# automl/CARL

Measured on AMD Instinct MI355X. Metric: env-steps/sec (whole node) at 65k parallel contexts, 1/2/4/8 MI355X, higher is better.
Workload: dtype f32

## Files before the change

carl_amd/csrc/carl_policy.hip:

```cpp
#include <hip/hip_runtime.h>

#include <cstdint>

#include "../../include/carl_amd.h"
#include "classic_control.hip.h"
#include "host_common.hpp"
#include "policy_host.hpp"
#include "policy_kernels.hip.h"
#include "policy_launch.hpp"

namespace carl_host {

int policy_set_floats(const carl_policy_t* p) {
  if (p->n_in < 1 || p->n_in > CARL_POLICY_MAX_IN || p->n_out < 1 || p->n_out > 4 || p->n_hidden < 0 ||
      p->n_hidden > CARL_POLICY_MAX_HIDDEN)
    return -1;
  for (int l = 0; l < p->n_hidden; ++l)
    if (p->width[l] < 1 || p->width[l] > CARL_POLICY_MAX_WIDTH) return -1;
  const int64_t total = (int64_t)policy_transform_offset(p) + 2 * (int64_t)p->n_in + 1;
  return (int)((total + 3) / 4 * 4);
}

int policy_transform_offset(const carl_policy_t* p) {
  int total = 0, prev = p->n_in;
// ... 72 lines not shown
    return fail(CARL_ERR_INVALID_ARGUMENT, "%s: io.row_pitch %d < n_lanes %d", who, io->row_pitch, b->n_lanes);
  if (!carl_host::staged_rows(b, io, 15))
    return fail(CARL_ERR_UNSUPPORTED, "%s: rows of %d lanes for %d lanes: the closed-loop rollout writes the staged layout "
                "only (pitch %% 16 == 0 and n_lanes %% 16 == 0 or pitch == carl_rollout_pitch(n_lanes), arrays on 16-byte "
                "boundaries)", who, io->row_pitch > 0 ? io->row_pitch : b->n_lanes, b->n_lanes);
  return 0;
}

int check_batch_and_policy(const char* who, const carl_batch_t* batch, const carl_policy_t* policy_host,
                           carl_family_info_t* fi) {
  if (batch == nullptr || policy_host == nullptr) return fail(CARL_ERR_INVALID_ARGUMENT, "%s: batch / policy is NULL", who);
  if (batch->family >= CARL_N_FAMILIES)
    return fail(CARL_ERR_INVALID_ARGUMENT, "%s: family %d is a Brax family -- the closed-loop rollout covers the "
                "classic-control families only", who, batch->family);
  if (int e = validate_batch(batch, who)) return e;
  if (int e = carl_family_info(batch->family, fi)) return e;
  return validate_policy(batch, policy_host, *fi, who);
}

}

int check_rollout_policy(const char* who, const carl_batch_t* batch, const carl_policy_t* policy_host,
                         const carl_step_io_t* io, int32_t n_steps, const carl_policy_summary_t* summary_out,
                         carl_family_info_t* fi) {
  if (int e = check_batch_and_policy(who, batch, policy_host, fi)) return e;
  if (n_steps < 0) return fail(CARL_ERR_INVALID_ARGUMENT, "%s: n_steps %d < 0", who, n_steps);
  if (io == nullptr) {
    if (summary_out == nullptr || !summary_out->episodes || !summary_out->return_sum || !summary_out->length_sum)
      return fail(CARL_ERR_INVALID_ARGUMENT, "%s: summary mode (io NULL) needs all three summary arrays", who);
  } else {
    if (int e = validate_io(batch, io, *fi, who)) return e;
    if (summary_out != nullptr && (!summary_out->episodes || !summary_out->return_sum || !summary_out->length_sum))
      return fail(CARL_ERR_INVALID_ARGUMENT, "%s: a summary needs all three arrays", who);
  }
  if (summary_out != nullptr && !(batch->flags & CARL_FLAG_AUTORESET))
    return fail(CARL_ERR_UNSUPPORTED, "%s: a summary needs CARL_FLAG_AUTORESET (without auto-reset a finished lane "
                "reports done on every later step, and its episode would be counted on each of them)", who);
  return 0;
}

int policy_rollout_without_steps(const char* who, const carl_batch_t* batch, const carl_policy_summary_t* summary_out,
                                 void* stream) {
  if (summary_out == nullptr || batch->n_lanes == 0) return 0;
  hipStream_t s = (hipStream_t)stream;
  const size_t bytes = (size_t)batch->n_lanes * 4;
  for (void* p : {(void*)summary_out->episodes, (void*)summary_out->return_sum, (void*)summary_out->length_sum})
    if (const hipError_t e = hipMemsetAsync(p, 0, bytes, s); e != hipSuccess)
      return fail((int)e, "%s: hipMemsetAsync: %s", who, hipGetErrorString(e));
  return 0;
}

int check_evaluate_policy(const char* who, const carl_batch_t* batch, const carl_policy_t* policy_host,
                          int32_t n_episodes, int32_t max_steps, const carl_policy_episodes_t* out,
                          carl_family_info_t* fi) {
  if (int e = check_batch_and_policy(who, batch, policy_host, fi)) return e;
  if (out == nullptr || !out->episodes || !out->steps || !out->ret || !out->length || !out->context_id ||
      !out->terminated)
    return fail(CARL_ERR_INVALID_ARGUMENT, "%s: out and all six of its arrays are required", who);
  if (n_episodes < 1) return fail(CARL_ERR_INVALID_ARGUMENT, "%s: n_episodes %d < 1", who, n_episodes);
  if (max_steps < 0) return fail(CARL_ERR_INVALID_ARGUMENT, "%s: max_steps %d < 0", who, max_steps);
  if ((int64_t)n_episodes * batch->n_lanes >= ((int64_t)1 << 31))
    return fail(CARL_ERR_INVALID_ARGUMENT, "%s: n_episodes %d x %d lanes records do not fit 2^31 - 1", who, n_episodes,
                batch->n_lanes);
  if (!(batch->flags & CARL_FLAG_AUTORESET))
    return fail(CARL_ERR_UNSUPPORTED, "%s: needs CARL_FLAG_AUTORESET (without auto-reset a finished lane reports done on "
                "every later step, and its episode would be counted on each of them)", who);
  return 0;
}

}

namespace {

using carl_host::launch_policy_kernel;
using carl_host::PolicyKernel;
using carl_host::with_padded_hidden;

template <class Fam>
int launch_policy(const carl_batch_t* b, const carl_policy_t* p, const carl_step_io_t* io, int n_steps,
                  const carl_policy_summary_t* sum, hipStream_t s) {
  const bool summary = io == nullptr;
  static_assert(carl::policy_lds_bytes<Fam, 64, false>() + carl::static_lds_bytes<Fam>() <= carl::kCuLdsBytes,
                "the closed-loop rollout's LDS does not fit a compute unit");
  const auto k = with_padded_hidden(carl_host::policy_padded_hidden(p), [&](auto h) {
    constexpr int H = decltype(h)::value;
    if (summary) return PolicyKernel{carl::policy_rollout_kernel<Fam, H, true>, carl::policy_lds_bytes<Fam, H, true>()};
    return PolicyKernel{carl::policy_rollout_kernel<Fam, H, false>, carl::policy_lds_bytes<Fam, H, false>()};
  });
  const int threads = summary ? carl::kPolicyThreadsSummary : carl::kPolicyThreadsTransitions;
  return launch_policy_kernel("carl_rollout_policy", k, b->n_lanes, threads, s, *b, carl_host::launch_io(b, io), *p,
                              carl_host::policy_set_floats(p), carl_host::launch_summary(sum), n_steps);
}

template <class Fam>
int launch_episodes(const carl_batch_t* b, const carl_policy_t* p, int n_episodes, int max_steps,
                    const carl_policy_episodes_t* out, hipStream_t s) {
  const auto k = with_padded_hidden(carl_host::policy_padded_hidden(p), [](auto h) {
    constexpr int H = decltype(h)::value;
    return PolicyKernel{carl::policy_episodes_kernel<Fam, H>, carl::policy_lds_bytes<Fam, H, true>()};
  });
  return launch_policy_kernel("carl_evaluate_policy", k, b->n_lanes, carl::kPolicyThreadsSummary, s, *b, *p,
                              carl_host::policy_set_floats(p), *out, n_episodes, max_steps);
}

}

extern "C" {

int32_t carl_policy_lane_quantum(void) { return carl::kPolicyLanes; }

int32_t carl_policy_set_floats(const carl_policy_t* policy_host) {
  if (policy_host == nullptr) return -1;
  return carl_host::policy_set_floats(policy_host);
}

int carl_rollout_policy(const carl_batch_t* batch, const carl_policy_t* policy_host, const carl_step_io_t* io,
                        int32_t n_steps, const carl_policy_summary_t* summary_out, void* stream) {
  const char* who = "carl_rollout_policy";
  carl_family_info_t fi;
  if (int e = carl_host::check_rollout_policy(who, batch, policy_host, io, n_steps, summary_out, &fi)) return e;
  if (batch->n_lanes == 0 || n_steps == 0) return carl_host::policy_rollout_without_steps(who, batch, summary_out, stream);
  return carl_host::with_classic_family(batch, [&](auto fam) {
    return launch_policy<decltype(fam)>(batch, policy_host, io, n_steps, summary_out, (hipStream_t)stream);
  });
}

int carl_evaluate_policy(const carl_batch_t* batch, const carl_policy_t* policy_host, int32_t n_episodes,
                         int32_t max_steps, const carl_policy_episodes_t* out, void* stream) {
  carl_family_info_t fi;
  if (int e = carl_host::check_evaluate_policy("carl_evaluate_policy", batch, policy_host, n_episodes, max_steps, out, &fi))
    return e;
  if (batch->n_lanes == 0) return 0;
  return carl_host::with_classic_family(batch, [&](auto fam) {
    return launch_episodes<decltype(fam)>(batch, policy_host, n_episodes, max_steps, out, (hipStream_t)stream);
  });
}

}
```

carl_amd/csrc/carl_policy_sample.hip:

```cpp
#include <hip/hip_runtime.h>

#include <cstdint>

#include "../../include/carl_amd.h"
#include "classic_control.hip.h"
#include "host_common.hpp"
#include "policy_host.hpp"
#include "policy_kernels.hip.h"
#include "policy_launch.hpp"

namespace carl_host {

int check_sampling(const char* who, const carl_policy_sampling_t* smp, const carl_family_info_t& fi, LogProb log_prob) {
  if (smp == nullptr) return fail(CARL_ERR_INVALID_ARGUMENT, "%s: sampling is NULL", who);
  if (!fi.action_is_discrete && smp->log_std == nullptr)
    return fail(CARL_ERR_INVALID_ARGUMENT, "%s: a Box family needs sampling->log_std ([n_sets] on the device)", who);
  if (log_prob == LogProb::kRefused && smp->log_prob != nullptr)
    return fail(CARL_ERR_INVALID_ARGUMENT, "%s: sampling->log_prob is a transitions-mode output (io != NULL); this mode "
                "stores nothing per step", who);
  if (log_prob == LogProb::kRequired && smp->log_prob == nullptr)
    return fail(CARL_ERR_INVALID_ARGUMENT, "%s: a sampled launch with a critic stores the log-probabilities: "
                "sampling->log_prob is NULL", who);
  if ((reinterpret_cast<uintptr_t>(smp->log_prob) & 15) != 0)
    return fail(CARL_ERR_UNSUPPORTED, "%s: sampling->log_prob is not on a 16-byte boundary", who);
  return 0;
}

}

namespace {

using carl_host::check_sampling;
using carl_host::launch_policy_kernel;
using carl_host::LogProb;
using carl_host::PolicyKernel;
using carl_host::with_padded_hidden;

template <class Fam>
int launch_sampled(const carl_batch_t* b, const carl_policy_t* p, const carl_policy_sampling_t* smp,
                   const carl_step_io_t* io, int n_steps, const carl_policy_summary_t* sum, hipStream_t s) {
  const bool summary = io == nullptr, logp = smp->log_prob != nullptr;
  static_assert(carl::policy_lds_bytes<Fam, 64, false, true>() + carl::static_lds_bytes<Fam>() <= carl::kCuLdsBytes,
                "the sampled rollout's LDS (the log_prob column included) does not fit a compute unit");
  const auto k = with_padded_hidden(carl_host::policy_padded_hidden(p), [&](auto h) {
    constexpr int H = decltype(h)::value;
    using carl::policy_lds_bytes;
    if (summary) return PolicyKernel{carl::policy_rollout_sampled_kernel<Fam, H, true, false>, policy_lds_bytes<Fam, H, true>()};
    if (logp)
      return PolicyKernel{carl::policy_rollout_sampled_kernel<Fam, H, false, true>, policy_lds_bytes<Fam, H, false, true>()};
    return PolicyKernel{carl::policy_rollout_sampled_kernel<Fam, H, false, false>, policy_lds_bytes<Fam, H, false>()};
  });
  const int threads = summary ? carl::kPolicyThreadsSummary : carl::kPolicyThreadsTransitions;
  return launch_policy_kernel("carl_rollout_policy_sampled", k, b->n_lanes, threads, s, *b, carl_host::launch_io(b, io), *p,
                              carl_host::policy_set_floats(p), carl_host::launch_summary(sum), n_steps, *smp);
}

template <class Fam>
int launch_sampled_episodes(const carl_batch_t* b, const carl_policy_t* p, const carl_policy_sampling_t* smp,
                            int n_episodes, int max_steps, const carl_policy_episodes_t* out, hipStream_t s) {
  const auto k = with_padded_hidden(carl_host::policy_padded_hidden(p), [](auto h) {
    constexpr int H = decltype(h)::value;
    return PolicyKernel{carl::policy_episodes_sampled_kernel<Fam, H>, carl::policy_lds_bytes<Fam, H, true>()};
  });
  return launch_policy_kernel("carl_evaluate_policy_sampled", k, b->n_lanes, carl::kPolicyThreadsSummary, s, *b, *p,
                              carl_host::policy_set_floats(p), *out, n_episodes, max_steps, *smp);
}

}

extern "C" {

int carl_rollout_policy_sampled(const carl_batch_t* batch, const carl_policy_t* policy_host,
                                const carl_policy_sampling_t* sampling, const carl_step_io_t* io, int32_t n_steps,
                                const carl_policy_summary_t* summary_out, void* stream) {
  const char* who = "carl_rollout_policy_sampled";
  carl_family_info_t fi;
  if (int e = carl_host::check_rollout_policy(who, batch, policy_host, io, n_steps, summary_out, &fi)) return e;
  if (int e = check_sampling(who, sampling, fi, io != nullptr ? LogProb::kOptional : LogProb::kRefused)) return e;
  if (batch->n_lanes == 0 || n_steps == 0) return carl_host::policy_rollout_without_steps(who, batch, summary_out, stream);
  return carl_host::with_classic_family(batch, [&](auto fam) {
    return launch_sampled<decltype(fam)>(batch, policy_host, sampling, io, n_steps, summary_out, (hipStream_t)stream);
  });
}

int carl_evaluate_policy_sampled(const carl_batch_t* batch, const carl_policy_t* policy_host,
                                 const carl_policy_sampling_t* sampling, int32_t n_episodes, int32_t max_steps,
                                 const carl_policy_episodes_t* out, void* stream) {
  const char* who = "carl_evaluate_policy_sampled";
  carl_family_info_t fi;
  if (int e = carl_host::check_evaluate_policy(who, batch, policy_host, n_episodes, max_steps, out, &fi)) return e;
  if (int e = check_sampling(who, sampling, fi, LogProb::kRefused)) return e;
  if (batch->n_lanes == 0) return 0;
  return carl_host::with_classic_family(batch, [&](auto fam) {
    return launch_sampled_episodes<decltype(fam)>(batch, policy_host, sampling, n_episodes, max_steps, out,
                                                  (hipStream_t)stream);
  });
}

}
```

carl_amd/csrc/engine_kernels.hip.h:

```cpp
#pragma once

#include <type_traits>

#include "carl_device.hip.h"


namespace carl {

template <bool LDS>
using ctx_t = std::conditional_t<LDS, LdsCtx, GlobalCtx>;

template <class Fam, class = void>
struct has_tables : std::false_type {};
template <class Fam>
struct has_tables<Fam, std::void_t<decltype(Fam::kUsesSinCosTab)>> : std::bool_constant<Fam::kUsesSinCosTab> {};

template <class Fam>
__device__ __forceinline__ void stage_family_tables() {
  if constexpr (has_tables<Fam>::value) {
    Fam::stage_tables();
    __syncthreads();
  }
}

// ... 613 lines not shown
    } else if constexpr (kU8) {
      return CARL_LD(reinterpret_cast<const unsigned int*>(p));
    } else if constexpr (kF16 || kBF16) {
      return CARL_LD(reinterpret_cast<const vu2*>(p));
    } else {
      const vi4* q = reinterpret_cast<const vi4*>(p);
      return Wide{CARL_LD(q), CARL_LD(q + 1)};
    }
#undef CARL_LD
  }
  __device__ static __forceinline__ LdsRow narrow(const R& r) {
    if constexpr (kSame || kNarrow) {
      return r;
    } else {
      return V{r.lo.x, r.lo.z, r.hi.x, r.hi.z};
    }
  }

  bool fast;

  __device__ __forceinline__ void issue(const AStore* __restrict__ act, size_t n, int cols, int lane_base, int l, int t0_,
                                        int n_steps) {
    t0 = t0_;
    fast = t0 + CHUNK <= n_steps;
    if constexpr (DEEP) {
      const int lane4 = min(lane_base + 4 * l, cols - 4);
      const int last = n_steps - 1;
      a0 = load_row(act + (size_t)min(t0, last) * n + lane4);
      a1 = load_row(act + (size_t)min(t0 + 1, last) * n + lane4);
      a2 = load_row(act + (size_t)min(t0 + 2, last) * n + lane4);
      a3 = load_row(act + (size_t)min(t0 + 3, last) * n + lane4);
      if constexpr (CHUNK == 8) {
        a4 = load_row(act + (size_t)min(t0 + 4, last) * n + lane4);
        a5 = load_row(act + (size_t)min(t0 + 5, last) * n + lane4);
        a6 = load_row(act + (size_t)min(t0 + 6, last) * n + lane4);
        a7 = load_row(act + (size_t)min(t0 + 7, last) * n + lane4);
      }
      return;
    }
    if (!fast) return;
    const int lane4 = min(lane_base + 4 * l, cols - 4);
    const AStore* row = act + (size_t)t0 * n;
    a0 = load_row(row + lane4);
    row += n;
    a1 = load_row(row + lane4);
    row += n;
    a2 = load_row(row + lane4);
    row += n;
    a3 = load_row(row + lane4);
    if constexpr (CHUNK == 8) {
      row += n;
      a4 = load_row(row + lane4);
      row += n;
      a5 = load_row(row + lane4);
      row += n;
      a6 = load_row(row + lane4);
      row += n;
      a7 = load_row(row + lane4);
    }
  }
  __device__ __forceinline__ void commit(LdsElem* buf, const AStore* __restrict__ act, size_t n, int cols, int lane_base, int l,
                                         int n_steps) const {
    LdsRow* dst = reinterpret_cast<LdsRow*>(buf + 4 * l);
    constexpr int row = kRolloutLanes / 4;
    if (fast || DEEP) {
      dst[0] = narrow(a0);
      dst[row] = narrow(a1);
      dst[2 * row] = narrow(a2);
      dst[3 * row] = narrow(a3);
      if constexpr (CHUNK == 8) {
        dst[4 * row] = narrow(a4);
        dst[5 * row] = narrow(a5);
        dst[6 * row] = narrow(a6);
        dst[7 * row] = narrow(a7);
      }
      return;
    }
    const AStore* src = act + (size_t)t0 * n + min(lane_base + 4 * l, cols - 4);
#pragma unroll 1
    for (int u = 0; u < CHUNK && t0 + u < n_steps; ++u) dst[u * row] = narrow(load_row(src + (size_t)u * n));
  }
};

template <class Fam>
__device__ __forceinline__ void drain_records(char* buf, const carl_step_io_t& io, size_t n, int cols, int lane_base, int l,
                                              int which, int t0, int steps) {
  using SK = LdsSink<Fam>;
  const int valid = min(kRolloutLanes, cols - lane_base);
  typedef float vf4 __attribute__((ext_vector_type(4)));
  auto put = [](char* dst, const char* src) {
    const vf4 v = *reinterpret_cast<const vf4*>(src);
    __builtin_nontemporal_store(v, reinterpret_cast<vf4*>(dst));
  };
  for (int u = which; u < steps; u += kStorers) {
    char* rec = buf + (size_t)u * SK::kStepBytes;
    const size_t row = (size_t)(t0 + u) * n + lane_base;
    char* g_obs = reinterpret_cast<char*>(io.obs + row * Fam::D);
    char* fl = rec + SK::kFlagOff + 16 * l;
    const int fl_lane = 16 * (l & 15);
    uint8_t* fl_dst = (l < 16) ? io.terminated + row + fl_lane : io.truncated + row + fl_lane;
    if (valid == kRolloutLanes) {
#pragma unroll
      for (int off = 0; off < SK::kObsBytes; off += 1024) put(g_obs + off + 16 * l, rec + off + 16 * l);
      put(reinterpret_cast<char*>(io.reward + row) + 16 * l, rec + SK::kObsBytes + 16 * l);
      if (l < 32) put(reinterpret_cast<char*>(fl_dst), fl);
    } else {
#pragma unroll
      for (int off = 0; off < SK::kObsBytes; off += 1024)
        if (off + 16 * l < valid * Fam::D * 4) put(g_obs + off + 16 * l, rec + off + 16 * l);
      if (16 * l < valid * 4) put(reinterpret_cast<char*>(io.reward + row) + 16 * l, rec + SK::kObsBytes + 16 * l);
      if (l < 32 && fl_lane < valid) put(reinterpret_cast<char*>(fl_dst), fl);
    }
    if (l < 32) *reinterpret_cast<vf4*>(fl) = vf4{0.0f, 0.0f, 0.0f, 0.0f};
  }
}

template <class Fam, int CHUNK>
__device__ __forceinline__ void zero_flag_rows(char* out_buf, int l, int which) {
  using SK = LdsSink<Fam>;
  typedef float vf4 __attribute__((ext_vector_type(4)));
  if (l < 32)
    for (int u = which; u < 2 * CHUNK; u += kStorers)
      *reinterpret_cast<vf4*>(out_buf + (size_t)u * SK::kStepBytes + SK::kFlagOff + 16 * l) = vf4{0.0f, 0.0f, 0.0f, 0.0f};
}

template <class Fam, class Ctx>
__device__ __forceinline__ void load_staged_lane(const carl_batch_t& b, const Ctx& ctx, int lane, bool active,
                                                 LaneRegs<Fam>& r) {
  const int src = min(lane, b.n_lanes - 1);
  load_lane<Fam>(b, ctx, src, r);
  if (!r.episode_valid) {
    r.episode = b.episode[src];
    r.episode_valid = true;
    settle(r.episode);
  }
  r.valid = active;
}

template <class Fam, int A64, bool PLAIN, bool LDSCTX, bool MOVES, bool FINAL, bool AR, int CHUNK, bool DEEPALL = false>
__device__ __forceinline__ void rollout_staged_body(const carl_batch_t& b, const carl_step_io_t& io, const int n_steps,
                                                    const int wg, float* lds_dyn) {
  constexpr int kStageChunk = CHUNK;
  stage_family_tables<Fam>();
  using AStore = action_store_t<Fam, A64>;
  using Action = typename Fam::Action;
  using SK = LdsSink<Fam>;
  constexpr bool kDeep = !std::is_same_v<AStore, long long> &&
                         (DEEPALL || (deep_action_prefetch_of<Fam>::value && !std::is_same_v<AStore, Action>));
  using Pipe = ActionPipe<AStore, Action, kStageChunk, kDeep>;
  using LdsAct = typename Pipe::LdsElem;
  LdsAct* act_buf = reinterpret_cast<LdsAct*>(lds_dyn);
  char* out_buf = reinterpret_cast<char*>(lds_dyn) + (size_t)2 * kStageChunk * kRolloutLanes * sizeof(float);
  float* ctx_lds = reinterpret_cast<float*>(out_buf + (size_t)2 * kStageChunk * SK::kStepBytes);
  const ctx_t<LDSCTX> ctx = make_ctx<LDSCTX, Fam::F>(b, ctx_lds);
  const int wave = __builtin_amdgcn_readfirstlane((int)(threadIdx.x / kWave));
  const int storer = wave - (kRolloutLanes / kWave + 1);
  const bool compute = wave < kRolloutLanes / kWave;
  const bool loader = wave == kRolloutLanes / kWave;
  const int hl = threadIdx.x % kWave;
  const int lane_base = wg * kRolloutLanes;
  const int lane = lane_base + (compute ? (int)threadIdx.x : 0);
  const bool active = compute && lane < b.n_lanes;
  const uint64_t glane = (uint64_t)(b.lane_offset + lane);
  const size_t n = (size_t)io.row_pitch;
  const int n_cols = (b.n_lanes + 15) & ~15;
  const int max_steps = b.max_episode_steps;
  const AStore* act = static_cast<const AStore*>(io.action);
  constexpr int kBufActs = kStageChunk * kRolloutLanes;
  LaneRegs<Fam> r{};
  Pipe pipe;
  [[maybe_unused]] Pipe pipe_b;
  float* const final_base = (io.final_obs != nullptr && active) ? io.final_obs + (size_t)lane * Fam::D : nullptr;
  if (!compute && !loader) zero_flag_rows<Fam, CHUNK>(out_buf, hl, storer);
  if (loader) {
    pipe.issue(act, n, n_cols, lane_base, hl, 0, n_steps);
    pipe.commit(act_buf, act, n, n_cols, lane_base, hl, n_steps);
    pipe.issue(act, n, n_cols, lane_base, hl, kStageChunk, n_steps);
    if constexpr (kDeep) pipe_b.issue(act, n, n_cols, lane_base, hl, 2 * kStageChunk, n_steps);
  } else if (compute) {
    load_staged_lane<Fam>(b, ctx, lane, active, r);
  }
  __syncthreads();
  auto run_role = [&](auto role_tag) -> int {
  constexpr int ROLE = decltype(role_tag)::value;
  if constexpr (ROLE == 1 && kDeep) {
    int lbuf = 0;
    for (int t0 = 0;;) {
      pipe.commit(act_buf + (lbuf ^ 1) * kBufActs, act, n, n_cols, lane_base, hl, n_steps);
      pipe.issue(act, n, n_cols, lane_base, hl, t0 + 3 * kStageChunk, n_steps);
      __syncthreads();
      lbuf ^= 1;
      if (t0 + kStageChunk >= n_steps) break;
      pipe_b.commit(act_buf + (lbuf ^ 1) * kBufActs, act, n, n_cols, lane_base, hl, n_steps);
      pipe_b.issue(act, n, n_cols, lane_base, hl, t0 + 4 * kStageChunk, n_steps);
      __syncthreads();
      lbuf ^= 1;
      t0 += 2 * kStageChunk;
      if (t0 >= n_steps) break;
    }
    return lbuf;
  }
  int buf = 0;
  [[maybe_unused]] DenseNext<Fam> nx{};
  [[maybe_unused]] const bool autoreset = (b.flags & CARL_FLAG_AUTORESET) != 0;
  [[maybe_unused]] const int max_steps_eff = max_steps > 0 ? max_steps : 0x7fffffff;
// ... 115 lines not shown
```

carl_amd/csrc/policy_kernels.hip.h:

```cpp
#pragma once

#include "engine_kernels.hip.h"

namespace carl {

constexpr int kPolicyLanes = kRolloutLanes;
constexpr int kPolicyThreadsSummary = kPolicyLanes;
constexpr int kPolicyThreadsTransitions = kPolicyLanes + kStorers * kWave;

template <class Fam>
struct policy_outputs : std::integral_constant<int, std::is_same_v<typename Fam::Action, float> ? 1
                                                    : (std::is_same_v<Fam, CartPole> ? 2 : 3)> {};

template <class Fam, int H>
struct PolicyLayout {
  static constexpr int K = (Fam::F + Fam::D + 3) / 4 * 4;
  static constexpr int HI = H == 0 ? K : H;
  static constexpr int kW1 = 0, kB1 = kW1 + H * K, kW2 = kB1 + H, kB2 = kW2 + H * H, kWh = kB2 + H, kBh = kWh + HI * 4;
  static constexpr int kShift = kBh + 4, kScale = kShift + K, kClip = kScale + K;
  static constexpr int kFloats = kClip + 4;
  static constexpr size_t kBytes = (size_t)kFloats * sizeof(float);
};

template <bool LOGP>
__host__ __device__ constexpr size_t policy_logp_lds_bytes(int chunk) {
  return LOGP ? (size_t)2 * chunk * kPolicyLanes * 4 : 0;
}
template <class Fam, bool LOGP = false>
__host__ __device__ constexpr int policy_chunk() {
  return rollout_staged_lds_bytes<Fam, 8>() + policy_logp_lds_bytes<LOGP>(8) + PolicyLayout<Fam, 64>::kBytes +
                     static_lds_bytes<Fam>() <= kCuLdsBytes ? 8 : 4;
}
template <class Fam, int H, bool SUMMARY, bool LOGP = false>
__host__ __device__ constexpr size_t policy_lds_bytes() {
  constexpr int CHUNK = policy_chunk<Fam, LOGP>();
  return PolicyLayout<Fam, H>::kBytes +
         (SUMMARY ? 0 : rollout_staged_lds_bytes<Fam, CHUNK>() + policy_logp_lds_bytes<LOGP>(CHUNK));
}

template <class Fam, int H>
__device__ __forceinline__ void stage_policy(float* w, const carl_policy_t& pol, int set_floats, int set) {
  using L = PolicyLayout<Fam, H>;
  const float* src = pol.params + (size_t)set * set_floats;
  const int n_in = pol.n_in, n_ctx = pol.n_ctx, n_out = pol.n_out;
  const int nh = pol.n_hidden;
  const int w0 = nh > 0 ? pol.width[0] : 0, w1 = nh > 1 ? pol.width[1] : 0;
  const int dims[CARL_POLICY_MAX_HIDDEN + 2] = {n_in, nh > 0 ? w0 : n_out, nh > 1 ? w1 : n_out, n_out};
  int p_w[CARL_POLICY_MAX_HIDDEN + 1] = {0, 0, 0}, p_b[CARL_POLICY_MAX_HIDDEN + 1] = {0, 0, 0};
  int off = 0;
#pragma unroll
  for (int l = 0; l <= CARL_POLICY_MAX_HIDDEN; ++l) {
    if (l <= nh) {
      p_w[l] = off;
      off += dims[l + 1] * dims[l];
      p_b[l] = off;
      off += dims[l + 1];
    }
  }
  const int p_w0 = p_w[0], p_b0 = p_b[0], p_w1 = p_w[1], p_b1 = p_b[1];
  const int p_shift = off, p_scale = p_shift + n_in, p_clip = p_scale + n_in;
  auto in_of = [&](int s) -> int {
    if (s < n_ctx) return s;
    if (s >= Fam::F && s < Fam::F + Fam::D) return n_ctx + (s - Fam::F);
    return -1;
  };
  const int hw = p_w[nh], hb = p_b[nh], hin = dims[nh];
  for (int e = threadIdx.x; e < L::kFloats; e += blockDim.x) {
    float v = 0.0f;
    if (e < L::kB1) {
      const int j = e / L::K, s = e % L::K, i = in_of(s);
      if (j < w0 && i >= 0) v = src[p_w0 + j * n_in + i];
    } else if (e < L::kW2) {
      const int j = e - L::kB1;
      if (j < w0) v = src[p_b0 + j];
    } else if (e < L::kB2) {
      const int j = (e - L::kW2) / (H > 0 ? H : 1), i = (e - L::kW2) % (H > 0 ? H : 1);
      if (j < w1 && i < w0) v = src[p_w1 + j * w0 + i];
    } else if (e < L::kWh) {
      const int j = e - L::kB2;
      if (j < w1) v = src[p_b1 + j];
    } else if (e < L::kBh) {
      const int j = (e - L::kWh) / 4, k = (e - L::kWh) % 4;
      const int i = H == 0 ? in_of(j) : (j < hin ? j : -1);
      if (k < n_out && i >= 0) v = src[hw + k * hin + i];
    } else if (e < L::kShift) {
      const int k = e - L::kBh;
      if (k < n_out) v = src[hb + k];
    } else if (e < L::kScale) {
      const int i = in_of(e - L::kShift);
      if (i >= 0) v = src[p_shift + i];
    } else if (e < L::kClip) {
      const int i = in_of(e - L::kScale);
      if (i >= 0) v = src[p_scale + i];
    } else {
      v = src[p_clip];
    }
    w[e] = v;
  }
}

typedef float pvf4 __attribute__((ext_vector_type(4)));

__device__ __forceinline__ pvf4 bcast4(const float* p) { return *reinterpret_cast<const pvf4*>(p); }

__device__ __forceinline__ float tanh_fast(float v) {
#pragma clang fp contract(off)
  const float e = __expf(2.0f * v);
  return 1.0f - __fdividef(2.0f, e + 1.0f);
}

template <int N>
__device__ __forceinline__ void activate(float (&h)[N], int act, int width) {
  if (act == CARL_POLICY_TANH) {
#pragma unroll
    for (int j = 0; j < N; ++j) h[j] = tanh_fast(h[j]);
  } else if (act == CARL_POLICY_RELU) {
#pragma unroll
    for (int j = 0; j < N; ++j) h[j] = fmaxf(h[j], 0.0f);
  }
  if (width < N) {
// ... 89 lines not shown
    return y[0];
  } else {
    int best = 0;
    float top = y[0];
#pragma unroll
    for (int k = 1; k < policy_outputs<Fam>::value; ++k) {
      const bool gt = y[k] > top;
      best = gt ? k : best;
      top = gt ? y[k] : top;
    }
    return best;
  }
}

template <class Fam>
struct ModePick {
  static constexpr bool kSampled = false, kLogProb = false;
};

template <class Fam, bool LOGP>
struct SampledPick {
  static constexpr bool kSampled = true, kLogProb = LOGP;
  uint64_t seed;
  float sigma;
  float lp0;

  static __device__ __forceinline__ SampledPick of(const carl_policy_sampling_t& smp, const carl_policy_t& pol) {
    SampledPick p{smp.seed, 1.0f, 0.0f};
    if constexpr (std::is_same_v<typename Fam::Action, float>) {
      const float ls = smp.log_std[(int)blockIdx.x * kPolicyLanes / pol.lanes_per_set];
      p.sigma = expf(ls);
      p.lp0 = -ls - 0.918938533204672742f;
    }
    return p;
  }

  template <int H>
  __device__ __forceinline__ typename Fam::Action choose(const float* w, const float (&x)[PolicyLayout<Fam, H>::K],
                                                         int n_hidden, int act, int w0, int w1, uint64_t glane,
                                                         const LaneRegs<Fam>& r, float& lp) const {
#pragma clang fp contract(off)
    const u32x4 wd = lane_words(seed, glane, r.episode - 1u, kSubSample | (uint32_t)r.elapsed);
    float y[4];
    if constexpr (std::is_same_v<typename Fam::Action, float>) {
      const float z = normal_from_words(wd.x, wd.y);
      policy_head<Fam, H>(w, x, n_hidden, act, w0, w1, y);
      if constexpr (LOGP) lp = __fmaf_rn(-0.5f * z, z, lp0);
      return __fmaf_rn(sigma, z, y[0]);
    } else {
      constexpr int NA = policy_outputs<Fam>::value;
      const float u = u01(wd.x);
      policy_head<Fam, H>(w, x, n_hidden, act, w0, w1, y);
      float m = y[0];
#pragma unroll
      for (int k = 1; k < NA; ++k) m = fmaxf(m, y[k]);
      float c[NA];
      float s = 0.0f;
#pragma unroll
      for (int k = 0; k < NA; ++k) c[k] = s = s + expf(y[k] - m);
      const float t = u * s;
      int a = NA - 1;
      float ya = y[NA - 1];
#pragma unroll
      for (int k = NA - 2; k >= 0; --k) {
        const bool in = t < c[k];
        a = in ? k : a;
        ya = in ? y[k] : ya;
      }
      if constexpr (LOGP) lp = (ya - m) - logf(s);
      return a;
    }
  }
};

template <class Fam>
struct NullSink {
  static constexpr bool kLazyFlags = true;
  __device__ __forceinline__ void put_reward(float) const {}
  __device__ __forceinline__ void put_flags(bool, bool) const {}
  __device__ __forceinline__ void put_obs(const float (&)[Fam::D]) const {}
  __device__ __forceinline__ float* final_obs_ptr() const { return nullptr; }
};

__device__ __forceinline__ void drain_actions(const char* buf, void* action, size_t n, int cols, int lane_base, int l,
                                              int which, int t0, int steps) {
  const int valid = min(kPolicyLanes, cols - lane_base);
  for (int u = which; u < steps; u += kStorers) {
    const char* src = buf + (size_t)u * kPolicyLanes * 4 + 16 * l;
    char* dst = reinterpret_cast<char*>(action) + ((size_t)(t0 + u) * n + lane_base) * 4 + 16 * l;
    if (4 * l < valid) __builtin_nontemporal_store(*reinterpret_cast<const pvf4*>(src), reinterpret_cast<pvf4*>(dst));
  }
}

template <class Fam, int H, bool SUMMARY>
__global__ void __launch_bounds__(SUMMARY ? kPolicyThreadsSummary : kPolicyThreadsTransitions)
    policy_rollout_kernel(const carl_batch_t b, const carl_step_io_t io, const carl_policy_t pol, const int set_floats,
                          const carl_policy_summary_t sum, const int n_steps) {
  using Pick = ModePick<Fam>;
  const Pick pick{};
  float* const log_prob = nullptr;
#include "policy_rollout_body.inc"
}

template <class Fam, int H, bool SUMMARY, bool LOGP>
__global__ void __launch_bounds__(SUMMARY ? kPolicyThreadsSummary : kPolicyThreadsTransitions)
    policy_rollout_sampled_kernel(const carl_batch_t b, const carl_step_io_t io, const carl_policy_t pol,
                                  const int set_floats, const carl_policy_summary_t sum, const int n_steps,
                                  const carl_policy_sampling_t smp) {
  static_assert(!(SUMMARY && LOGP), "a summary stores no per-step column");
  using Pick = SampledPick<Fam, LOGP>;
  const Pick pick = Pick::of(smp, pol);
  float* const log_prob = smp.log_prob;
#include "policy_rollout_body.inc"
}

template <class Fam>
struct TermSink {
  static constexpr bool kLazyFlags = true;
  bool* te;
  __device__ __forceinline__ void put_reward(float) const {}
  __device__ __forceinline__ void put_flags(bool t, bool) const { *te = t; }
  __device__ __forceinline__ void put_obs(const float (&)[Fam::D]) const {}
  __device__ __forceinline__ float* final_obs_ptr() const { return nullptr; }
};

template <class Fam, int H>
struct NoInputStats {
  static constexpr bool kOn = false;
};

template <class Fam, int H>
__global__ void __launch_bounds__(kPolicyThreadsSummary)
    policy_episodes_kernel(const carl_batch_t b, const carl_policy_t pol, const int set_floats,
                           const carl_policy_episodes_t ep, const int n_episodes, const int max_steps) {
  using Pick = ModePick<Fam>;
  const Pick pick{};
  using Stats = NoInputStats<Fam, H>;
  [[maybe_unused]] Stats istats;
#include "policy_episodes_body.inc"
}

template <class Fam, int H>
__global__ void __launch_bounds__(kPolicyThreadsSummary)
    policy_episodes_sampled_kernel(const carl_batch_t b, const carl_policy_t pol, const int set_floats,
                                   const carl_policy_episodes_t ep, const int n_episodes, const int max_steps,
                                   const carl_policy_sampling_t smp) {
  using Pick = SampledPick<Fam, false>;
  const Pick pick = Pick::of(smp, pol);
  using Stats = NoInputStats<Fam, H>;
  [[maybe_unused]] Stats istats;
#include "policy_episodes_body.inc"
}

}
```

carl_amd/csrc/policy_launch.hpp:

```cpp
#pragma once

#include <hip/hip_runtime.h>

#include <cstddef>
#include <type_traits>

#include "../../include/carl_amd.h"
#include "host_common.hpp"
#include "policy_kernels.hip.h"

namespace carl_host {

template <class Fn>
auto with_padded_hidden(int H, Fn&& fn) {
  return H == 0    ? fn(std::integral_constant<int, 0>{})
         : H == 32 ? fn(std::integral_constant<int, 32>{})
                   : fn(std::integral_constant<int, 64>{});
}

template <class... P>
struct PolicyKernel {
  void (*fn)(P...);
  size_t lds;
};
template <class... P>
PolicyKernel(void (*)(P...), size_t) -> PolicyKernel<P...>;

inline int policy_workgroups(int32_t n_lanes) {
  return n_lanes <= 0 ? 0 : (n_lanes + carl::kPolicyLanes - 1) / carl::kPolicyLanes;
}

template <class... P>
int launch_policy_kernel(const char* who, PolicyKernel<P...> k, int32_t n_lanes, int threads, hipStream_t s,
                         const P&... args) {
  if (int e = ensure_dynamic_lds(reinterpret_cast<const void*>(k.fn), k.lds, who)) return e;
  hipLaunchKernelGGL(k.fn, dim3(policy_workgroups(n_lanes)), dim3(threads), k.lds, s, args...);
  return check_launch(who);
}

inline carl_step_io_t launch_io(const carl_batch_t* b, const carl_step_io_t* io) {
  carl_step_io_t r{};
  if (io != nullptr) {
    r = *io;
    r.row_pitch = io->row_pitch > 0 ? io->row_pitch : b->n_lanes;
  }
  return r;
}

inline carl_policy_summary_t launch_summary(const carl_policy_summary_t* sum) {
  return sum != nullptr ? *sum : carl_policy_summary_t{nullptr, nullptr, nullptr};
}

inline carl_policy_sampling_t launch_sampling(const carl_policy_sampling_t* smp) {
  return smp != nullptr ? *smp : carl_policy_sampling_t{0, nullptr, nullptr};
}

}
```

carl_amd/csrc/policy_rollout_body.inc:

```
  using L = PolicyLayout<Fam, H>;
  using SK = LdsSink<Fam>;
  using Action = typename Fam::Action;
  constexpr int CHUNK = policy_chunk<Fam, Pick::kLogProb>();
  extern __shared__ float lds_dyn[];
  stage_family_tables<Fam>();
  float* const wts = lds_dyn;
  char* const out_buf = reinterpret_cast<char*>(lds_dyn) + L::kBytes;
  char* const act_buf = out_buf + (size_t)2 * CHUNK * SK::kStepBytes;
  char* const lp_buf = act_buf + (size_t)2 * CHUNK * kPolicyLanes * 4;
  const int lane_base = (int)blockIdx.x * kPolicyLanes;
  stage_policy<Fam, H>(wts, pol, set_floats, lane_base / pol.lanes_per_set);
  const GlobalCtx ctx{b.ctx_table, b.ctx_stride};
  const int wave = __builtin_amdgcn_readfirstlane((int)(threadIdx.x / kWave));
  const bool compute = wave < kPolicyLanes / kWave;
  const int hl = threadIdx.x % kWave;
  const int storer = wave - kPolicyLanes / kWave;
  const int lane = lane_base + (compute ? (int)threadIdx.x : 0);
  const bool active = compute && lane < b.n_lanes;
  const uint64_t glane = (uint64_t)(b.lane_offset + lane);
  const size_t n = (size_t)io.row_pitch;
  const int n_cols = (b.n_lanes + 15) & ~15;
  if (!SUMMARY && !compute) zero_flag_rows<Fam, CHUNK>(out_buf, hl, storer);
  __syncthreads();

  if (compute) {
    LaneRegs<Fam> r{};
    load_staged_lane<Fam>(b, ctx, lane, active, r);
    float* const final_base = (!SUMMARY && io.final_obs != nullptr && active) ? io.final_obs + (size_t)lane * Fam::D : nullptr;
    const int n_ctx = pol.n_ctx, n_hidden = pol.n_hidden, act = pol.activation;
    const int w0 = pol.width[0], w1 = pol.width[1];
    const float clip = wts[L::kClip];
    float x[L::K];
#pragma unroll
    for (int s = 0; s < L::K; ++s) x[s] = 0.0f;
    int x_cidx = -1;
    int ep_count = 0, len_sum = 0;
    float ret_sum = 0.0f;
    int buf = 0;
    for (int t0 = 0; t0 < n_steps; t0 += CHUNK, buf ^= 1) {
      const int steps = min(CHUNK, n_steps - t0);
      if constexpr (predraw_of<Fam>::value) predraw<Fam>(b, glane, r);
      char* const rec = out_buf + (size_t)buf * CHUNK * SK::kStepBytes;
      Action* const my_act = reinterpret_cast<Action*>(act_buf + (size_t)buf * CHUNK * kPolicyLanes * 4) + threadIdx.x;
#pragma unroll 1
      for (int u = 0; u < steps; ++u) {
        if (ballot(r.cidx != x_cidx) != 0ull) {
#pragma unroll
          for (int k = 0; k < Fam::F; ++k)
            if (k < n_ctx) x[k] = normalize_input(ctx.get(pol.ctx_rows[k], r.cidx), wts[L::kShift + k], wts[L::kScale + k], clip);
          x_cidx = r.cidx;
        }
        float o[Fam::D];
        Fam::observe(r.s, r.aux, o);
#pragma unroll
        for (int d = 0; d < Fam::D; ++d)
          x[Fam::F + d] = normalize_input(o[d], wts[L::kShift + Fam::F + d], wts[L::kScale + Fam::F + d], clip);
        [[maybe_unused]] float lp;
        Action a;
        if constexpr (Pick::kSampled)
          a = pick.template choose<H>(wts, x, n_hidden, act, w0, w1, glane, r, lp);
        else
          a = policy_action<Fam, H>(wts, x, n_hidden, act, w0, w1);
        const int before = r.n_new_episodes;
        if constexpr (SUMMARY) {
          step_lane<Fam, GlobalCtx, true, NullSink<Fam>>(b, ctx, NullSink<Fam>{}, b.max_episode_steps, true, lane, glane,
                                                          a, r);
        } else {
          my_act[u * kPolicyLanes] = a;
          if constexpr (Pick::kLogProb)
            reinterpret_cast<float*>(lp_buf + (size_t)buf * CHUNK * kPolicyLanes * 4)[u * kPolicyLanes + threadIdx.x] = lp;
          const SK sink{rec + (size_t)u * SK::kStepBytes, final_base, n * Fam::D, t0 + u, (int)threadIdx.x};
          step_lane<Fam, GlobalCtx, true, SK>(b, ctx, sink, b.max_episode_steps, true, lane, glane, a, r);
        }
        const bool fin = r.n_new_episodes != before;
        ep_count += fin ? 1 : 0;
        len_sum += fin ? r.fin_length : 0;
        ret_sum = fin ? ret_sum + r.fin_return : ret_sum;
      }
      if constexpr (!SUMMARY) __syncthreads();
    }
    if (active) {
      store_lane<Fam>(b, ctx, lane, r);
      if (sum.episodes != nullptr) {
        sum.episodes[lane] = ep_count;
        sum.return_sum[lane] = ret_sum;
        sum.length_sum[lane] = len_sum;
      }
    }
  } else if constexpr (!SUMMARY) {
    int buf = 0;
    for (int t0 = 0; t0 < n_steps; t0 += CHUNK, buf ^= 1) {
      if (t0 > 0) {
        drain_records<Fam>(out_buf + (size_t)(buf ^ 1) * CHUNK * SK::kStepBytes, io, n, n_cols, lane_base, hl, storer,
                           t0 - CHUNK, CHUNK);
        drain_actions(act_buf + (size_t)(buf ^ 1) * CHUNK * kPolicyLanes * 4, const_cast<void*>(io.action), n, n_cols,
                      lane_base, hl, storer, t0 - CHUNK, CHUNK);
        if constexpr (Pick::kLogProb)
          drain_actions(lp_buf + (size_t)(buf ^ 1) * CHUNK * kPolicyLanes * 4, log_prob, n, n_cols, lane_base, hl,
                        storer, t0 - CHUNK, CHUNK);
      }
      __syncthreads();
    }
    if (n_steps > 0) {
      const int last_t0 = ((n_steps - 1) / CHUNK) * CHUNK;
      drain_records<Fam>(out_buf + (size_t)(buf ^ 1) * CHUNK * SK::kStepBytes, io, n, n_cols, lane_base, hl, storer,
                         last_t0, n_steps - last_t0);
      drain_actions(act_buf + (size_t)(buf ^ 1) * CHUNK * kPolicyLanes * 4, const_cast<void*>(io.action), n, n_cols,
                    lane_base, hl, storer, last_t0, n_steps - last_t0);
      if constexpr (Pick::kLogProb)
        drain_actions(lp_buf + (size_t)(buf ^ 1) * CHUNK * kPolicyLanes * 4, log_prob, n, n_cols, lane_base, hl, storer,
                      last_t0, n_steps - last_t0);
    }
  }
```

Measured before the change: 239.1 billion.

## Drain rollout records inline from compute waves for the 64-wide hidden policy

For policies padded to hidden width 64, the transitions-mode rollout now uses a new kernel variant with no dedicated storer waves. The compute waves write each chunk to a single LDS buffer, synchronise, and drain records, actions and log-probs to global memory themselves. This halves the staging LDS and shrinks the block, which should let more blocks fit on a compute unit. The cost is that compute and global stores no longer overlap within a block, and each chunk takes an extra barrier.

```diff
diff --git a/carl_amd/csrc/carl_policy.hip b/carl_amd/csrc/carl_policy.hip
--- a/carl_amd/csrc/carl_policy.hip
+++ b/carl_amd/csrc/carl_policy.hip
@@ -178,12 +178,16 @@
   const bool summary = io == nullptr;
   static_assert(carl::policy_lds_bytes<Fam, 64, false>() + carl::static_lds_bytes<Fam>() <= carl::kCuLdsBytes,
                 "the closed-loop rollout's LDS does not fit a compute unit");
-  const auto k = with_padded_hidden(carl_host::policy_padded_hidden(p), [&](auto h) {
+  const int padded = carl_host::policy_padded_hidden(p);
+  const auto k = with_padded_hidden(padded, [&](auto h) {
     constexpr int H = decltype(h)::value;
     if (summary) return PolicyKernel{carl::policy_rollout_kernel<Fam, H, true>, carl::policy_lds_bytes<Fam, H, true>()};
-    return PolicyKernel{carl::policy_rollout_kernel<Fam, H, false>, carl::policy_lds_bytes<Fam, H, false>()};
-  });
-  const int threads = summary ? carl::kPolicyThreadsSummary : carl::kPolicyThreadsTransitions;
+    if constexpr (carl_host::policy_drains_inline(H))
+      return PolicyKernel{carl::policy_rollout_inline_kernel<Fam, H>, carl::policy_lds_bytes<Fam, H, false, false, true>()};
+    else
+      return PolicyKernel{carl::policy_rollout_kernel<Fam, H, false>, carl::policy_lds_bytes<Fam, H, false>()};
+  });
+  const int threads = carl_host::policy_rollout_threads(summary, padded);
   return launch_policy_kernel("carl_rollout_policy", k, b->n_lanes, threads, s, *b, carl_host::launch_io(b, io), *p,
                               carl_host::policy_set_floats(p), carl_host::launch_summary(sum), n_steps);
 }
diff --git a/carl_amd/csrc/carl_policy_sample.hip b/carl_amd/csrc/carl_policy_sample.hip
--- a/carl_amd/csrc/carl_policy_sample.hip
+++ b/carl_amd/csrc/carl_policy_sample.hip
@@ -42,15 +42,24 @@
   const bool summary = io == nullptr, logp = smp->log_prob != nullptr;
   static_assert(carl::policy_lds_bytes<Fam, 64, false, true>() + carl::static_lds_bytes<Fam>() <= carl::kCuLdsBytes,
                 "the sampled rollout's LDS (the log_prob column included) does not fit a compute unit");
-  const auto k = with_padded_hidden(carl_host::policy_padded_hidden(p), [&](auto h) {
+  const int padded = carl_host::policy_padded_hidden(p);
+  const auto k = with_padded_hidden(padded, [&](auto h) {
     constexpr int H = decltype(h)::value;
     using carl::policy_lds_bytes;
     if (summary) return PolicyKernel{carl::policy_rollout_sampled_kernel<Fam, H, true, false>, policy_lds_bytes<Fam, H, true>()};
-    if (logp)
-      return PolicyKernel{carl::policy_rollout_sampled_kernel<Fam, H, false, true>, policy_lds_bytes<Fam, H, false, true>()};
-    return PolicyKernel{carl::policy_rollout_sampled_kernel<Fam, H, false, false>, policy_lds_bytes<Fam, H, false>()};
+    if constexpr (carl_host::policy_drains_inline(H)) {
+      if (logp)
+        return PolicyKernel{carl::policy_rollout_sampled_inline_kernel<Fam, H, true>,
+                            policy_lds_bytes<Fam, H, false, true, true>()};
+      return PolicyKernel{carl::policy_rollout_sampled_inline_kernel<Fam, H, false>,
+                          policy_lds_bytes<Fam, H, false, false, true>()};
+    } else {
+      if (logp)
+        return PolicyKernel{carl::policy_rollout_sampled_kernel<Fam, H, false, true>, policy_lds_bytes<Fam, H, false, true>()};
+      return PolicyKernel{carl::policy_rollout_sampled_kernel<Fam, H, false, false>, policy_lds_bytes<Fam, H, false>()};
+    }
   });
-  const int threads = summary ? carl::kPolicyThreadsSummary : carl::kPolicyThreadsTransitions;
+  const int threads = carl_host::policy_rollout_threads(summary, padded);
   return launch_policy_kernel("carl_rollout_policy_sampled", k, b->n_lanes, threads, s, *b, carl_host::launch_io(b, io), *p,
                               carl_host::policy_set_floats(p), carl_host::launch_summary(sum), n_steps, *smp);
 }
diff --git a/carl_amd/csrc/engine_kernels.hip.h b/carl_amd/csrc/engine_kernels.hip.h
--- a/carl_amd/csrc/engine_kernels.hip.h
+++ b/carl_amd/csrc/engine_kernels.hip.h
@@ -719,7 +719,7 @@
   }
 };
 
-template <class Fam>
+template <class Fam, int WAVES = kStorers>
 __device__ __forceinline__ void drain_records(char* buf, const carl_step_io_t& io, size_t n, int cols, int lane_base, int l,
                                               int which, int t0, int steps) {
   using SK = LdsSink<Fam>;
@@ -729,7 +729,7 @@
     const vf4 v = *reinterpret_cast<const vf4*>(src);
     __builtin_nontemporal_store(v, reinterpret_cast<vf4*>(dst));
   };
-  for (int u = which; u < steps; u += kStorers) {
+  for (int u = which; u < steps; u += WAVES) {
     char* rec = buf + (size_t)u * SK::kStepBytes;
     const size_t row = (size_t)(t0 + u) * n + lane_base;
     char* g_obs = reinterpret_cast<char*>(io.obs + row * Fam::D);
@@ -752,12 +752,12 @@
   }
 }
 
-template <class Fam, int CHUNK>
+template <class Fam, int CHUNK, int WAVES = kStorers, int BUFS = 2>
 __device__ __forceinline__ void zero_flag_rows(char* out_buf, int l, int which) {
   using SK = LdsSink<Fam>;
   typedef float vf4 __attribute__((ext_vector_type(4)));
   if (l < 32)
-    for (int u = which; u < 2 * CHUNK; u += kStorers)
+    for (int u = which; u < BUFS * CHUNK; u += WAVES)
       *reinterpret_cast<vf4*>(out_buf + (size_t)u * SK::kStepBytes + SK::kFlagOff + 16 * l) = vf4{0.0f, 0.0f, 0.0f, 0.0f};
 }
 
diff --git a/carl_amd/csrc/policy_kernels.hip.h b/carl_amd/csrc/policy_kernels.hip.h
--- a/carl_amd/csrc/policy_kernels.hip.h
+++ b/carl_amd/csrc/policy_kernels.hip.h
@@ -7,6 +7,8 @@
 constexpr int kPolicyLanes = kRolloutLanes;
 constexpr int kPolicyThreadsSummary = kPolicyLanes;
 constexpr int kPolicyThreadsTransitions = kPolicyLanes + kStorers * kWave;
+constexpr int kPolicyThreadsInline = kPolicyLanes;
+constexpr int kPolicyWaves = kPolicyLanes / kWave;
 
 template <class Fam>
 struct policy_outputs : std::integral_constant<int, std::is_same_v<typename Fam::Action, float> ? 1
@@ -31,11 +33,11 @@
   return rollout_staged_lds_bytes<Fam, 8>() + policy_logp_lds_bytes<LOGP>(8) + PolicyLayout<Fam, 64>::kBytes +
                      static_lds_bytes<Fam>() <= kCuLdsBytes ? 8 : 4;
 }
-template <class Fam, int H, bool SUMMARY, bool LOGP = false>
+template <class Fam, int H, bool SUMMARY, bool LOGP = false, bool INLINE = false>
 __host__ __device__ constexpr size_t policy_lds_bytes() {
   constexpr int CHUNK = policy_chunk<Fam, LOGP>();
   return PolicyLayout<Fam, H>::kBytes +
-         (SUMMARY ? 0 : rollout_staged_lds_bytes<Fam, CHUNK>() + policy_logp_lds_bytes<LOGP>(CHUNK));
+         (SUMMARY ? 0 : (rollout_staged_lds_bytes<Fam, CHUNK>() + policy_logp_lds_bytes<LOGP>(CHUNK)) / (INLINE ? 2 : 1));
 }
 
 template <class Fam, int H>
@@ -291,10 +293,11 @@
   __device__ __forceinline__ float* final_obs_ptr() const { return nullptr; }
 };
 
+template <int WAVES = kStorers>
 __device__ __forceinline__ void drain_actions(const char* buf, void* action, size_t n, int cols, int lane_base, int l,
                                               int which, int t0, int steps) {
   const int valid = min(kPolicyLanes, cols - lane_base);
-  for (int u = which; u < steps; u += kStorers) {
+  for (int u = which; u < steps; u += WAVES) {
     const char* src = buf + (size_t)u * kPolicyLanes * 4 + 16 * l;
     char* dst = reinterpret_cast<char*>(action) + ((size_t)(t0 + u) * n + lane_base) * 4 + 16 * l;
     if (4 * l < valid) __builtin_nontemporal_store(*reinterpret_cast<const pvf4*>(src), reinterpret_cast<pvf4*>(dst));
@@ -308,6 +311,18 @@
   using Pick = ModePick<Fam>;
   const Pick pick{};
   float* const log_prob = nullptr;
+  constexpr bool INLINE_DRAIN = false;
+#include "policy_rollout_body.inc"
+}
+
+template <class Fam, int H>
+__global__ void __launch_bounds__(kPolicyThreadsInline)
+    policy_rollout_inline_kernel(const carl_batch_t b, const carl_step_io_t io, const carl_policy_t pol,
+                                 const int set_floats, const carl_policy_summary_t sum, const int n_steps) {
+  using Pick = ModePick<Fam>;
+  const Pick pick{};
+  float* const log_prob = nullptr;
+  constexpr bool SUMMARY = false, INLINE_DRAIN = true;
 #include "policy_rollout_body.inc"
 }
 
@@ -320,6 +335,19 @@
   using Pick = SampledPick<Fam, LOGP>;
   const Pick pick = Pick::of(smp, pol);
   float* const log_prob = smp.log_prob;
+  constexpr bool INLINE_DRAIN = false;
+#include "policy_rollout_body.inc"
+}
+
+template <class Fam, int H, bool LOGP>
+__global__ void __launch_bounds__(kPolicyThreadsInline)
+    policy_rollout_sampled_inline_kernel(const carl_batch_t b, const carl_step_io_t io, const carl_policy_t pol,
+                                         const int set_floats, const carl_policy_summary_t sum, const int n_steps,
+                                         const carl_policy_sampling_t smp) {
+  using Pick = SampledPick<Fam, LOGP>;
+  const Pick pick = Pick::of(smp, pol);
+  float* const log_prob = smp.log_prob;
+  constexpr bool SUMMARY = false, INLINE_DRAIN = true;
 #include "policy_rollout_body.inc"
 }
 
diff --git a/carl_amd/csrc/policy_launch.hpp b/carl_amd/csrc/policy_launch.hpp
--- a/carl_amd/csrc/policy_launch.hpp
+++ b/carl_amd/csrc/policy_launch.hpp
@@ -16,6 +16,12 @@
   return H == 0    ? fn(std::integral_constant<int, 0>{})
          : H == 32 ? fn(std::integral_constant<int, 32>{})
                    : fn(std::integral_constant<int, 64>{});
+}
+
+constexpr bool policy_drains_inline(int H) { return H == 64; }
+inline int policy_rollout_threads(bool summary, int H) {
+  return summary ? carl::kPolicyThreadsSummary
+                 : policy_drains_inline(H) ? carl::kPolicyThreadsInline : carl::kPolicyThreadsTransitions;
 }
 
 template <class... P>
diff --git a/carl_amd/csrc/policy_rollout_body.inc b/carl_amd/csrc/policy_rollout_body.inc
--- a/carl_amd/csrc/policy_rollout_body.inc
+++ b/carl_amd/csrc/policy_rollout_body.inc
@@ -2,17 +2,19 @@
   using SK = LdsSink<Fam>;
   using Action = typename Fam::Action;
   constexpr int CHUNK = policy_chunk<Fam, Pick::kLogProb>();
+  constexpr int BUFS = INLINE_DRAIN ? 1 : 2;
+  static_assert(!(SUMMARY && INLINE_DRAIN), "a summary drains nothing");
   extern __shared__ float lds_dyn[];
   stage_family_tables<Fam>();
   float* const wts = lds_dyn;
   char* const out_buf = reinterpret_cast<char*>(lds_dyn) + L::kBytes;
-  char* const act_buf = out_buf + (size_t)2 * CHUNK * SK::kStepBytes;
-  char* const lp_buf = act_buf + (size_t)2 * CHUNK * kPolicyLanes * 4;
+  char* const act_buf = out_buf + (size_t)BUFS * CHUNK * SK::kStepBytes;
+  char* const lp_buf = act_buf + (size_t)BUFS * CHUNK * kPolicyLanes * 4;
   const int lane_base = (int)blockIdx.x * kPolicyLanes;
   stage_policy<Fam, H>(wts, pol, set_floats, lane_base / pol.lanes_per_set);
   const GlobalCtx ctx{b.ctx_table, b.ctx_stride};
   const int wave = __builtin_amdgcn_readfirstlane((int)(threadIdx.x / kWave));
-  const bool compute = wave < kPolicyLanes / kWave;
+  const bool compute = INLINE_DRAIN || wave < kPolicyLanes / kWave;
   const int hl = threadIdx.x % kWave;
   const int storer = wave - kPolicyLanes / kWave;
   const int lane = lane_base + (compute ? (int)threadIdx.x : 0);
@@ -20,7 +22,10 @@
   const uint64_t glane = (uint64_t)(b.lane_offset + lane);
   const size_t n = (size_t)io.row_pitch;
   const int n_cols = (b.n_lanes + 15) & ~15;
-  if (!SUMMARY && !compute) zero_flag_rows<Fam, CHUNK>(out_buf, hl, storer);
+  if constexpr (INLINE_DRAIN)
+    zero_flag_rows<Fam, CHUNK, kPolicyWaves, BUFS>(out_buf, hl, wave);
+  else if (!SUMMARY && !compute)
+    zero_flag_rows<Fam, CHUNK>(out_buf, hl, storer);
   __syncthreads();
 
   if (compute) {
@@ -37,7 +42,7 @@
     int ep_count = 0, len_sum = 0;
     float ret_sum = 0.0f;
     int buf = 0;
-    for (int t0 = 0; t0 < n_steps; t0 += CHUNK, buf ^= 1) {
+    for (int t0 = 0; t0 < n_steps; t0 += CHUNK, buf ^= BUFS - 1) {
       const int steps = min(CHUNK, n_steps - t0);
       if constexpr (predraw_of<Fam>::value) predraw<Fam>(b, glane, r);
       char* const rec = out_buf + (size_t)buf * CHUNK * SK::kStepBytes;
@@ -77,7 +82,16 @@
         len_sum += fin ? r.fin_length : 0;
         ret_sum = fin ? ret_sum + r.fin_return : ret_sum;
       }
-      if constexpr (!SUMMARY) __syncthreads();
+      if constexpr (INLINE_DRAIN) {
+        __syncthreads();
+        drain_records<Fam, kPolicyWaves>(rec, io, n, n_cols, lane_base, hl, wave, t0, steps);
+        drain_actions<kPolicyWaves>(act_buf, const_cast<void*>(io.action), n, n_cols, lane_base, hl, wave, t0, steps);
+        if constexpr (Pick::kLogProb)
+          drain_actions<kPolicyWaves>(lp_buf, log_prob, n, n_cols, lane_base, hl, wave, t0, steps);
+        __syncthreads();
+      } else if constexpr (!SUMMARY) {
+        __syncthreads();
+      }
     }
     if (active) {
       store_lane<Fam>(b, ctx, lane, r);
@@ -87,7 +101,7 @@
         sum.length_sum[lane] = len_sum;
       }
     }
-  } else if constexpr (!SUMMARY) {
+  } else if constexpr (!SUMMARY && !INLINE_DRAIN) {
     int buf = 0;
     for (int t0 = 0; t0 < n_steps; t0 += CHUNK, buf ^= 1) {
       if (t0 > 0) {
```

After: 236.3 billion. 1.2% lower.
